# anyboby/Constrained-Model-Based-Policy-Optimization

Hardware: AMD Instinct MI355X
Metric: imagined env-steps/sec (ensemble rollout) + CPO update ms (higher is better)
Workload: dtype f32; 1 GPU; AntSafe-v2 imagined rollout: E=7 x (37->512->512->60) swish ensemble, 5 elites, 3+3 critics 128x128, tanh policy 128x128, B=100000 branches/GPU, maxroll 35 (34 steps), fixed-horizon mode, reset->sample*->finish_all_paths->get(); rollout_mode=schedule, branches_per_gpu=100000, branches_total=100000, horizon=34, task=AntSafe-v2

## Files before the change

constrained-model-based-policy-optimization_amd/csrc/critic_f16.hip:

```cpp
#include "common.h"
#include "ens_mlp_internal.h"
#include "f16_split.h"
#include "policy_f16_tile.h"

namespace {

constexpr int HC = 128;
constexpr int NT = HC / 32;
constexpr int S1 = HC / 16;

struct CfNet {
  const f16x8 *w0, *w1;
  size_t w0_stride, w1_stride;
  const float *b0, *b1, *w2, *b2;
  const float *cst;
  size_t w2_stride;
  const float *stats;
  const float *in_mu, *in_sig, *out_mu, *out_sig;
  float *out;
};

struct CfArgs {
  CfNet net[2];
  const float *obs;
// ... 218 lines not shown
    const int n2 = tid / KP, k = tid - n2 * KP;
    const CfNet &M = a.net[n2];
    const int kc = k < a.obs_dim ? k : 0;
    s_mu[n2 * KP + k] = (M.in_mu && k < a.obs_dim) ? M.in_mu[kc] : 0.0f;
    s_sig[n2 * KP + k] = (M.in_mu && k < a.obs_dim) ? 1.0f / M.in_sig[kc] : 1.0f;
  }
  __syncthreads();
  for (int base = 0; base < tiles * 32 * KP; base += 512 * 4) {
    float xv[4];
    bool ok[4];
#pragma unroll
    for (int u = 0; u < 4; ++u) {
      const int i = base + 512 * u + tid, b = i / KP, k = i - b * KP;
      const int rr = i < tiles * 32 * KP ? rows[b] : -1;
      xv[u] = a.obs[(size_t)(rr >= 0 ? rr : 0) * a.obs_dim + (k < a.obs_dim ? k : 0)];
      ok[u] = rr >= 0 && k < a.obs_dim;
    }
#pragma unroll
    for (int u = 0; u < 4; ++u) {
      const int i = base + 512 * u + tid, b = i / KP, k = i - b * KP;
      if (i < tiles * 32 * KP) xraw[b * XS + k] = ok[u] ? xv[u] : 0.0f;
    }
  }
  for (int net = 0; net < 2 * E; ++net) {
    const int ni = net / E, e = net - ni * E;
    const CfNet &N = a.net[ni];
    __syncthreads();
    {
      const f16x8 *g0 = N.w0 + (size_t)e * N.w0_stride, *g1 = N.w1 + (size_t)e * N.w1_stride;
      constexpr int TOT = G::W0Q + G::W1Q;
      for (int base = 0; base < TOT; base += 512 * 5) {
        f16x8 q[5];
#pragma unroll
        for (int u = 0; u < 5; ++u) {
          const int i = base + 512 * u + tid;
          const int ic = i < TOT ? i : 0;
          q[u] = ic < G::W0Q ? g0[ic] : g1[ic - G::W0Q];
        }
#pragma unroll
        for (int u = 0; u < 5; ++u) {
          const int i = base + 512 * u + tid;
          if (i < TOT) w0s[i] = q[u];
        }
      }
    }
    __syncthreads();
    const float *st = N.stats + (size_t)e * NSTAT;
    const f16x8 *w0 = w0s + lane, *w1 = w1s + lane;
    for (int t = wave; t < tiles; t += 8) {
      const float *xt = xraw + (size_t)t * 32 * XS;
      float xs[S0][8];
      float m0 = 0.0f;
#pragma unroll
      for (int s = 0; s < S0; ++s)
#pragma unroll
        for (int j = 0; j < 8; ++j) {
          const int k = 16 * s + 8 * hh + j;
          float x = (xt[r * XS + k] - s_mu[ni * KP + k]) * s_sig[ni * KP + k];
          if (k >= a.obs_dim) x = 0.0f;
          xs[s][j] = x;
          m0 = fmaxf(m0, fabsf(x));
        }
      m0 = fmaxf(m0, __shfl_xor(m0, 32, 64));
      const float t0 = pow2_lift(m0);
      const float bound1 = (st[1] * m0 + st[2]) * 1.001f, t1 = pow2_lift(bound1);
      const float inv0 = pow2_rcp(st[0] * t0), inv1 = pow2_rcp(st[4] * t1);
      f32x16 acc[NT];
#pragma unroll
      for (int tt = 0; tt < NT; ++tt)
// ... 173 lines not shown
    n.out = outs[i];
  }
  a.obs = d_obs; a.obs_dim = obs_dim; a.ensemble = v->ensemble;
  a.row_idx = d_row_idx; a.n_rows_dev = d_n_rows; a.n_rows = n_rows;
  const int S0 = ms[0]->h3_s0;
  a.has_pol = 0;
  if (policy != nullptr) {
    CMBPO_REQUIRE(cmbpo_internal_critic_pair_can_ride(v, vc, policy) && d_eps && d_pi && d_logp && d_mu && d_ls,
                  "critic pair: the actor cannot ride along (shape / path) or a NULL buffer");
    int ps0 = 0;
    if (int rc = cmbpo_internal_policy_f16_args(policy, &a.pol, &ps0, s)) return rc;
    CMBPO_REQUIRE(ps0 == S0, "critic pair: actor and critics disagree on the input slabs (%d, %d)", ps0, S0);
    a.pol.obs = d_obs; a.pol.eps = d_eps; a.pol.row_idx = d_row_idx; a.pol.n_rows_dev = d_n_rows; a.pol.n_rows = n_rows;
    a.pol.pi = d_pi; a.pol.logp = d_logp; a.pol.mu = d_mu; a.pol.ls = d_ls;
    a.has_pol = 1;
  }
  a.has_store = 0;
  if (store_vec != nullptr) {
    CMBPO_REQUIRE(d_row_idx != nullptr && n_rows < kCriticBigMin && store_vec->fin_code,
                  "critic pair: the store rides with the one-wave-per-member kernel on a row list only");
    a.sv = *store_vec;
    a.has_store = 1;
  }
  if (!a.has_pol && n_rows >= kCriticBigMin) {
    const int n_cu = cmbpo_cu_count();
    auto launch_big = [&](auto geo, auto kern) -> int {
      using G = decltype(geo);
      if (int rc = cmbpo_grant_lds(kern, G::LDS)) return rc;
      int ch = (cmbpo_ceil_div(n_rows, n_cu) + 31) / 32 * 32;
      if (ch > G::CH) ch = G::CH;
      hipLaunchKernelGGL(kern, dim3(cmbpo_ceil_div(n_rows, ch)), dim3(512), G::LDS, s, a, ch);
      CMBPO_HIP_CHECK(hipGetLastError());
      return CMBPO_OK;
    };
    if (S0 == 2) return launch_big(BigGeo<2>{}, critic_big_kernel<2>);
    if (S0 == 3) return launch_big(BigGeo<3>{}, critic_big_kernel<3>);
    return launch_big(BigGeo<4>{}, critic_big_kernel<4>);
  }
  const int threads = 64 * (2 * v->ensemble + a.has_pol);
  const size_t lds = ((size_t)32 * (16 * S0 + 1) + (size_t)2 * v->ensemble * 32) * sizeof(float);
  const int grid = cmbpo_ceil_div(n_rows, 32);
  if (S0 == 2) hipLaunchKernelGGL(critic_pair_kernel<2>, dim3(grid), dim3(threads), lds, s, a);
  else if (S0 == 3) hipLaunchKernelGGL(critic_pair_kernel<3>, dim3(grid), dim3(threads), lds, s, a);
  else hipLaunchKernelGGL(critic_pair_kernel<4>, dim3(grid), dim3(threads), lds, s, a);
  CMBPO_HIP_CHECK(hipGetLastError());
  return CMBPO_OK;
}
// ... 1 lines not shown
```

constrained-model-based-policy-optimization_amd/csrc/policy_f16_tile.h:

```cpp
#pragma once
#include "common.h"
#include "f16_split.h"

namespace {


constexpr int HP = 128;
constexpr int NTP = HP / 32;
constexpr int SP1 = HP / 16;
constexpr float T_H = 16384.0f;

struct PfArgs {
  const f16x8 *w0, *w1, *w2;
  const float *b0, *b1, *b2, *log_std, *stats;
  const float *obs, *eps;
  int obs_dim, act_dim;
  const int32_t *row_idx, *n_rows_dev;
  int n_rows;
  float *pi, *logp, *mu, *ls;
};

__device__ __forceinline__ void tanh_split4(const f32x16 &d, int q, float inv, const f32x4 &bv, unsigned (&q1)[2], unsigned (&q2)[2]) {
  float h[4];
#pragma unroll
  for (int i = 0; i < 4; ++i) h[i] = cmbpo_fast_tanh(__builtin_fmaf(d[4 * q + i], inv, bv[i]));
  split2<true>(h[0], h[1], T_H, q1[0], q2[0]);
  split2<true>(h[2], h[3], T_H, q1[1], q2[1]);
}

struct NoStage { __device__ void operator()() const {} };
template <int S0, bool STAGED, class STAGE = NoStage>
__device__ __forceinline__ void policy_tile(const PfArgs &a, int row0, int n_rows, float *xraw, int *rows, int lane,
                                            STAGE &&stage = STAGE()) {
  constexpr int KP = 16 * S0;
  const int r = lane & 31, hh = lane >> 5;
  const f16x8 *w0 = a.w0 + lane, *w1 = a.w1 + lane, *w2 = a.w2 + lane;
  constexpr int RW = S0 <= 2 ? 3 : 2;
  f16x8 A0[S0][NTP][2], R[3][NTP][2];
  auto load_w = [&](f16x8 (&x)[NTP][2], const f16x8 *w, int slabs, int s) {
#pragma unroll
    for (int t = 0; t < NTP; ++t) {
      const f16x8 *q = w + IMAGE_INDEX(t, slabs, s, 2, 0);
      x[t][0] = q[0]; x[t][1] = q[kImageLanes];
    }
  };
#pragma unroll
  for (int s = 0; s < S0; ++s) load_w(A0[s], w0, S0, s);
#pragma unroll
  for (int s = 0; s < RW; ++s) load_w(R[s], w1, SP1, s);
  if constexpr (!STAGED) {
    if (lane < 32) {
      const int rr = row0 + lane;
      int v = rr < n_rows ? rr : 0;
      if (a.row_idx) v = a.row_idx[v];
      rows[lane] = rr < n_rows ? v : -1;
    }
    __builtin_amdgcn_wave_barrier();
    for (int base = 0; base < 32 * KP; base += 64 * 8) {
      float xv[8];
      bool ok[8];
#pragma unroll
      for (int u = 0; u < 8; ++u) {
        const int i = base + 64 * u + lane, b = i / KP, k = i - b * KP;
        const int rr = rows[b];
        xv[u] = a.obs[(size_t)(rr >= 0 ? rr : 0) * a.obs_dim + (k < a.obs_dim ? k : 0)];
        ok[u] = rr >= 0 && k < a.obs_dim;
      }
#pragma unroll
      for (int u = 0; u < 8; ++u) {
        const int i = base + 64 * u + lane, b = i / KP, k = i - b * KP;
        xraw[b * (KP + 1) + k] = ok[u] ? xv[u] : 0.0f;
      }
// ... 14 lines not shown
      xs[s][j] = x;
      m0 = fmaxf(m0, fabsf(x));
    }
  m0 = fmaxf(m0, __shfl_xor(m0, 32, 64));
  const float t0 = pow2_lift(m0);
  const float inv0 = pow2_rcp(st[0] * t0), inv1 = pow2_rcp(st[4] * T_H), inv2 = pow2_rcp(st[8] * T_H);

  f32x16 acc[NTP];
  auto zero_acc = [&]() {
#pragma unroll
    for (int t = 0; t < NTP; ++t)
#pragma unroll
      for (int i = 0; i < 16; ++i) acc[t][i] = 0.0f;
  };
  zero_acc();
#pragma unroll
  for (int s = 0; s < S0; ++s) {
    unsigned c1[4], c2[4];
#pragma unroll
    for (int j = 0; j < 4; ++j) split2<true>(xs[s][2 * j], xs[s][2 * j + 1], t0, c1[j], c2[j]);
    const u32x4 u1 = {c1[0], c1[1], c1[2], c1[3]}, u2 = {c2[0], c2[1], c2[2], c2[3]};
    const f16x8 b1 = __builtin_bit_cast(f16x8, u1), b2 = __builtin_bit_cast(f16x8, u2);
#pragma unroll
    for (int t = 0; t < NTP; ++t) mm3(acc[t], A0[s][t][0], A0[s][t][1], b1, b2);
  }
  f16x8 bf[SP1][2];
  auto to_frags = [&](const float *bias, float inv) {
    u32x4 bu[SP1][2];
#pragma unroll
    for (int t = 0; t < NTP; ++t)
#pragma unroll
      for (int q = 0; q < 4; ++q) {
        const f32x4 bv = *reinterpret_cast<const f32x4 *>(bias + 32 * t + 8 * q + 4 * hh);
        unsigned q1[2], q2[2];
        tanh_split4(acc[t], q, inv, bv, q1, q2);
        const int S = 2 * t + (q >> 1), o = 2 * (q & 1);
        bu[S][0][o] = q1[0]; bu[S][0][o + 1] = q1[1];
        bu[S][1][o] = q2[0]; bu[S][1][o + 1] = q2[1];
      }
#pragma unroll
    for (int S = 0; S < SP1; ++S) { bf[S][0] = __builtin_bit_cast(f16x8, bu[S][0]); bf[S][1] = __builtin_bit_cast(f16x8, bu[S][1]); }
  };
  to_frags(a.b0, inv0);
  zero_acc();
  if constexpr (RW < 3) load_w(R[2], w1, SP1, 2);
#pragma unroll
  for (int s = 0; s < SP1; ++s) {
#pragma unroll
    for (int t = 0; t < NTP; ++t) mm3(acc[t], R[s % 3][t][0], R[s % 3][t][1], bf[s][0], bf[s][1]);
    if (s + 3 < SP1) load_w(R[s % 3], w1, SP1, s + 3);
  }
  f16x8 W2[SP1][2];
#pragma unroll
  for (int s = 0; s < SP1; ++s) { W2[s][0] = w2[IMAGE_INDEX(0, SP1, s, 2, 0)]; W2[s][1] = w2[IMAGE_INDEX(0, SP1, s, 2, 1)]; }
  to_frags(a.b1, inv1);
  f32x16 o;
#pragma unroll
  for (int i = 0; i < 16; ++i) o[i] = 0.0f;
#pragma unroll
  for (int s = 0; s < SP1; ++s) mm3(o, W2[s][0], W2[s][1], bf[s][0], bf[s][1]);
  const int rr = rows[r];
  const int A = a.act_dim;
  const int nq = (A + 7) >> 3;
  const size_t rbase = (size_t)(rr >= 0 ? rr : 0) * A;
  float lp = 0.0f;
#pragma unroll
  for (int q = 0; q < 4; ++q) {
    if (q < nq) {
      float ev[4], bv[4], lv[4];
#pragma unroll
      for (int e = 0; e < 4; ++e) {
        const int ac = 8 * q + 4 * hh + e, acc = ac < A ? ac : A - 1;
        ev[e] = a.eps[rbase + acc];
// ... 30 lines not shown
```

constrained-model-based-policy-optimization_amd/csrc/rollout_internal.h:

```cpp
#pragma once
#include "common.h"

int cmbpo_internal_book_post_mirror(const cmbpo_rollout_t *r, int n_alive, uint32_t *d_host_out, uint32_t seq, int spec, int min_alive,
                                    double stop_total, void *stream);
int cmbpo_internal_scalars_mirror(const cmbpo_rollout_t *r, uint32_t *d_host_out, uint32_t seq, void *stream);
int cmbpo_internal_book_pre(const cmbpo_rollout_t *r, int n_alive, int spec, int with_vec, void *stream);
int cmbpo_internal_store_nostats(const cmbpo_rollout_t *r, void *stream);
int cmbpo_internal_finish_post_fold(const cmbpo_rollout_t *r, void *stream);
int cmbpo_internal_spec_words(const cmbpo_rollout_t *r, int begin, void *stream);
```

constrained-model-based-policy-optimization_amd/csrc/rollout_state.hip:

```cpp
#include "common.h"
#include "rollout_internal.h"
#include <type_traits>

#include <math.h>

namespace {

constexpr int kScanThreads = 1024;

__device__ __forceinline__ int wave_incl_scan(int v, int lane) {
#pragma unroll
  for (int o = 1; o < 64; o <<= 1) {
    const int t = __shfl_up(v, o, 64);
    if (lane >= o) v += t;
  }
  return v;
}

__device__ __forceinline__ int block_excl_scan(int v, int *sm, int *total) {
  const int lane = threadIdx.x & 63, w = threadIdx.x >> 6, nw = (blockDim.x + 63) >> 6;
  const int inc = wave_incl_scan(v, lane);
  __syncthreads();
  if (lane == 63) sm[w] = inc;
  __syncthreads();
// ... 179 lines not shown
  for (int t = L - 1; t >= 0; --t) {
    const size_t o = (size_t)t * B + b;
    const float rw = r.rew_buf[o], v = r.val_buf[o], c = r.cost_buf[o], cv = r.cval_buf[o];
    double delta;
    if (zero_boot) {
      delta = __dsub_rn(__dadd_rn((double)rw, __dmul_rn(r.gamma, (double)vnext)), (double)v);
    } else {
      delta = (double)__fsub_rn(__fadd_rn(rw, __fmul_rn(g32, vnext)), v);
    }
    const float cdelta = __fsub_rn(__fadd_rn(c, __fmul_rn(cg32, cvnext)), cv);
    y = __dadd_rn(delta, __dmul_rn(gl, y));
    cy = __dadd_rn((double)cdelta, __dmul_rn(cgl, cy));
    const float adv = (float)y, cadv = (float)cy;
    r.adv_buf[o] = adv;
    r.ret_buf[o] = __fadd_rn(adv, v);
    r.cadv_buf[o] = cadv;
    r.cret_buf[o] = __fadd_rn(cadv, cv);
    vnext = v;
    cvnext = cv;
  }
  r.alive[b] = 0;
}

__device__ __forceinline__ void store_stats_body(const cmbpo_rollout_t &r);
__global__ __launch_bounds__(256) void finish_kernel(const cmbpo_rollout_t r, int mode, int fold_stats) {
  if (fold_stats && blockIdx.x == 0) store_stats_body(r);
  const int i = blockIdx.x * blockDim.x + threadIdx.x;
  const int n = r.iscal[CMBPO_I_N_ALIVE];
  if (i >= n) return;
  const int b = r.alive_idx[i];
  float lv, lcv;
  bool zero_boot = false;
  if (mode == 0) {
    const uint8_t code = r.fin_code[b];
    if (!code) return;
    lv = r.v_t[b];
    lcv = r.vc_t[b];
    if (code == 2) {
      lv = 0.0f;
      zero_boot = true;
    }
  } else if (mode == 1) {
    if (r.fin_code[b]) return;
    const bool horizon = (r.ptr + 1 >= r.max_path_length - 1);
    if (horizon) {
      lv = r.v_n[b];
    } else if (r.term_t[b]) {
      lv = 0.0f;
      zero_boot = true;
    } else {
      return;
    }
    lcv = r.vc_n[b];
    atomicAdd(&r.iscal[CMBPO_I_N_FIN_POST], 1);
  } else {
    if (!r.alive[b]) return;
    lv = r.v_t[b];
    lcv = r.vc_t[b];
  }
  gae_finish_path(r, b, lv, lcv, zero_boot);
}

constexpr int kStoreRows = 64;

__global__ __launch_bounds__(256) void store_kernel(const cmbpo_rollout_t r) {
  __shared__ int s_slot[kStoreRows];
  const int n = r.iscal[CMBPO_I_N_ALIVE];
  const int tid = threadIdx.x;
  const int row0 = blockIdx.x * kStoreRows;
  if (row0 >= n) return;
  const size_t B = (size_t)r.B;
  const int D = r.obs_dim, A = r.act_dim;
  if (tid < kStoreRows) {
    double a_cnt = 0, a_cost = 0, a_rew = 0, a_v = 0, a_vc = 0, a_epv = 0, a_maxdkl = 0, a_maxret = 0;
    const int i = row0 + tid;
    int b = -1;
    if (i < n) {
      b = r.alive_idx[i];
      if (r.fin_code[b]) b = -1;
    }
    s_slot[tid] = b;
    if (b >= 0) {
      const size_t col = (size_t)r.ptr * B + b;
      const float rw = r.rew_t[b], c = r.cost_t[b], v = r.v_t[b], vc = r.vc_t[b];
      const float epv = r.epv_t[b], dk = r.dkl_t[b];
      r.rew_buf[col] = rw;
      r.val_buf[col] = v;
      r.cost_buf[col] = c;
      r.cval_buf[col] = vc;
      r.logp_buf[col] = r.logp_t[b];
      r.len[b] = r.ptr + 1;
      const double pr = r.path_ret[b] + (double)rw;
      r.path_ret[b] = pr;
      r.path_cost[b] += (double)c;
      r.path_dyn_var[b] += (double)epv;
      r.dkl_acc[b] += (double)dk;
      a_cnt = 1.0; a_cost = c; a_rew = rw; a_v = v; a_vc = vc;
      a_epv = (double)epv * D;
      a_maxdkl = (double)dk;
      a_maxret = pr;
    }
    const double v0 = wave_sum(a_cnt), v1 = wave_sum(a_cost), v2 = wave_sum(a_rew), v3 = wave_sum(a_v);
    const double v4 = wave_sum(a_vc), v5 = wave_sum(a_epv), v6 = wave_max(a_maxdkl), v7 = wave_max(a_maxret);
    if (tid == 0) {
      double *dst = r.store_part + (size_t)blockIdx.x * 8;
      dst[0] = v0; dst[1] = v1; dst[2] = v2; dst[3] = v3; dst[4] = v4; dst[5] = v5; dst[6] = v6; dst[7] = v7;
    }
  }
  __syncthreads();
  const int rows_here = min(kStoreRows, n - row0);
  const float *vsrc[4] = {r.cur_obs, r.act_t, r.mu_t, r.ls_t};
  float *vdst[4] = {r.obs_buf, r.act_buf, r.mu_buf, r.ls_buf};
  const int vdim[4] = {D, A, A, A};
#pragma unroll
  for (int f = 0; f < 4; ++f) {
    const int dim = vdim[f];
    const float inv = 1.0f / (float)dim;
    for (int e = tid; e < rows_here * dim; e += 256) {
      const int k = (int)(((float)e + 0.5f) * inv);
      const int d = e - k * dim;
      const int b = s_slot[k];
      if (b >= 0) vdst[f][((size_t)r.ptr * B + b) * dim + d] = vsrc[f][(size_t)b * dim + d];
    }
  }
}

__device__ __forceinline__ void store_stats_body(const cmbpo_rollout_t &r) {
  __shared__ double sm_d[16];
  const int n = r.iscal[CMBPO_I_N_ALIVE];
// ... 11 lines not shown
  for (int k = 0; k < 6; ++k) s[k] = block_sum(t[k], sm_d);
  s[6] = block_max(t[6], sm_d);
  s[7] = block_max(t[7], sm_d);
  if (threadIdx.x == 0 && s[0] > 0.0) {
    const double cnt = s[0];
    const double dkl_mean = r.dscal[CMBPO_D_DKL_SUM_T] / (double)n;
    r.iscal[CMBPO_I_N_STORED] += (int)cnt;
    r.iscal[CMBPO_I_SIZE] += (int)cnt;
    r.dscal[CMBPO_D_TOTAL_SAMPLES] += cnt;
    r.dscal[CMBPO_D_TOTAL_COST] += s[1];
    r.dscal[CMBPO_D_TOTAL_REW] += s[2];
    r.dscal[CMBPO_D_SUM_PATH_RET] += s[2];
    r.dscal[CMBPO_D_SUM_PATH_COST] += s[1];
    r.dscal[CMBPO_D_TOTAL_VS] += s[3];
    r.dscal[CMBPO_D_TOTAL_CVS] += s[4];
    r.dscal[CMBPO_D_TOTAL_DYN_EP_VAR] += s[5];
    r.dscal[CMBPO_D_TOTAL_DKL] += dkl_mean * cnt;
    r.dscal[CMBPO_D_MAX_DKL] = fmax(r.dscal[CMBPO_D_MAX_DKL], s[6]);
    r.dscal[CMBPO_D_MAX_PATH_RETURN] = fmax(r.dscal[CMBPO_D_MAX_PATH_RETURN], s[7]);
  }
}

__global__ __launch_bounds__(256) void store_stats_kernel(const cmbpo_rollout_t r) { store_stats_body(r); }

constexpr int kBookMax = 1024;

__global__ __launch_bounds__(kScanThreads) void book_pre_kernel(const cmbpo_rollout_t r, int spec) {
  __shared__ int sm_i[17];
  __shared__ double sm_d[16];
  __shared__ double sm_m[8 * 16];
  __shared__ int s_unc;
  const int tid = threadIdx.x;
  if (spec && r.iscal[CMBPO_I_HALT]) return;
  const int n = r.iscal[CMBPO_I_N_ALIVE];
  {
    double c = 0.0, d = 0.0;
    for (int i = tid; i < n; i += kScanThreads) {
      const int b = r.alive_idx[i];
      const bool u = too_uncertain(r, b);
      r.fin_code[b] = u ? 1 : 0;
      c += u ? 1.0 : 0.0;
      d += (double)r.dkl_t[b];
    }
    double cd[2] = {c, d};
    block_reduce_many<2, 0>(cd, sm_m);
    c = cd[0]; d = cd[1];
// ... 656 lines not shown
extern "C" int cmbpo_rollout_finish(const cmbpo_rollout_t *r, int mode, void *stream) {
  if (int rc = check_rollout(r, "cmbpo_rollout_finish")) return rc;
  CMBPO_REQUIRE(mode >= 0 && mode <= 2, "cmbpo_rollout_finish: bad mode %d", mode);
  CMBPO_REQUIRE(r->rew_buf && r->val_buf && r->cost_buf && r->cval_buf && r->adv_buf && r->ret_buf &&
                    r->cadv_buf && r->cret_buf,
                "cmbpo_rollout_finish: NULL buffer");
  if (mode == 1) CMBPO_REQUIRE(r->v_n && r->vc_n && r->term_t, "cmbpo_rollout_finish: POST needs v_n, vc_n, term_t");
  else CMBPO_REQUIRE(r->v_t && r->vc_t, "cmbpo_rollout_finish: needs v_t, vc_t");
  hipLaunchKernelGGL(finish_kernel, dim3(cmbpo_ceil_div(r->B, 256)), dim3(256), 0, (hipStream_t)stream, *r, mode, 0);
  CMBPO_HIP_CHECK(hipGetLastError());
  return CMBPO_OK;
}

extern "C" int cmbpo_rollout_store(const cmbpo_rollout_t *r, void *stream) {
  if (int rc = check_rollout(r, "cmbpo_rollout_store")) return rc;
  CMBPO_REQUIRE(r->ptr < r->T, "cmbpo_rollout_store: buffer full (ptr %d == T)", r->ptr);
  CMBPO_REQUIRE(r->cur_obs && r->act_t && r->logp_t && r->mu_t && r->ls_t && r->v_t && r->vc_t && r->rew_t &&
                    r->cost_t && r->dkl_t && r->epv_t,
                "cmbpo_rollout_store: NULL step array");
  CMBPO_REQUIRE(r->obs_buf && r->act_buf && r->mu_buf && r->ls_buf && r->rew_buf && r->val_buf && r->cost_buf &&
                    r->cval_buf && r->logp_buf,
                "cmbpo_rollout_store: NULL buffer");
  CMBPO_REQUIRE(r->store_part != nullptr, "cmbpo_rollout_store: NULL store_part scratch");
  hipLaunchKernelGGL(store_kernel, dim3(cmbpo_ceil_div(r->B, kStoreRows)), dim3(256), 0, (hipStream_t)stream, *r);
  hipLaunchKernelGGL(store_stats_kernel, dim3(1), dim3(256), 0, (hipStream_t)stream, *r);
  CMBPO_HIP_CHECK(hipGetLastError());
  return CMBPO_OK;
}

int cmbpo_internal_store_nostats(const cmbpo_rollout_t *r, void *stream) {
  if (int rc = check_rollout(r, "cmbpo_rollout_store")) return rc;
  CMBPO_REQUIRE(r->ptr < r->T, "cmbpo_rollout_store: buffer full (ptr %d == T)", r->ptr);
  CMBPO_REQUIRE(r->cur_obs && r->act_t && r->logp_t && r->mu_t && r->ls_t && r->v_t && r->vc_t && r->rew_t && r->cost_t && r->dkl_t &&
                    r->epv_t && r->obs_buf && r->act_buf && r->mu_buf && r->ls_buf && r->rew_buf && r->val_buf && r->cost_buf &&
                    r->cval_buf && r->logp_buf && r->store_part,
                "cmbpo_rollout_store: NULL array");
  hipLaunchKernelGGL(store_kernel, dim3(cmbpo_ceil_div(r->B, kStoreRows)), dim3(256), 0, (hipStream_t)stream, *r);
  CMBPO_HIP_CHECK(hipGetLastError());
  return CMBPO_OK;
}
int cmbpo_internal_finish_post_fold(const cmbpo_rollout_t *r, void *stream) {
  if (int rc = check_rollout(r, "cmbpo_rollout_finish")) return rc;
  CMBPO_REQUIRE(r->v_n && r->vc_n && r->term_t && r->rew_buf && r->val_buf && r->cost_buf && r->cval_buf && r->adv_buf && r->ret_buf &&
                    r->cadv_buf && r->cret_buf && r->store_part,
                "cmbpo_rollout_finish (POST): NULL array");
  hipLaunchKernelGGL(finish_kernel, dim3(cmbpo_ceil_div(r->B, 256)), dim3(256), 0, (hipStream_t)stream, *r, 1, 1);
  CMBPO_HIP_CHECK(hipGetLastError());
  return CMBPO_OK;
}

extern "C" int cmbpo_rollout_book_pre_max_rows(void) { return kBookMax; }

extern "C" int cmbpo_rollout_book_pre(const cmbpo_rollout_t *r, int n_alive, void *stream) {
  if (int rc = check_rollout(r, "cmbpo_rollout_book_pre")) return rc;
  CMBPO_REQUIRE(n_alive >= 0 && n_alive <= kBookMax, "cmbpo_rollout_book_pre: %d alive rows, at most %d", n_alive, kBookMax);
  CMBPO_REQUIRE(!r->use_host_budget, "cmbpo_rollout_book_pre: the cross-shard budget exchange uses the separate kernels");
  CMBPO_REQUIRE(r->ptr < r->T, "cmbpo_rollout_book_pre: buffer full (ptr %d == T)", r->ptr);
  CMBPO_REQUIRE(r->dkl_t && r->dkl_acc && r->cur_obs && r->act_t && r->logp_t && r->mu_t && r->ls_t && r->v_t && r->vc_t &&
                    r->rew_t && r->cost_t && r->epv_t,
                "cmbpo_rollout_book_pre: NULL step array");
  CMBPO_REQUIRE(r->obs_buf && r->act_buf && r->mu_buf && r->ls_buf && r->rew_buf && r->val_buf && r->cost_buf && r->cval_buf &&
                    r->logp_buf && r->adv_buf && r->ret_buf && r->cadv_buf && r->cret_buf,
                "cmbpo_rollout_book_pre: NULL buffer");
  if (n_alive == 0) return CMBPO_OK;
  hipLaunchKernelGGL(book_pre_kernel, dim3(1), dim3(kScanThreads), 0, (hipStream_t)stream, *r, 0);
  hipLaunchKernelGGL(store_vec_kernel, dim3(cmbpo_ceil_div(n_alive, kStoreRows)), dim3(256), 0, (hipStream_t)stream, *r, 0);
  CMBPO_HIP_CHECK(hipGetLastError());
// ... 12 lines not shown
    hipLaunchKernelGGL(store_vec_kernel, dim3(cmbpo_ceil_div(n_alive, kStoreRows)), dim3(256), 0, (hipStream_t)stream, *r, spec);
  CMBPO_HIP_CHECK(hipGetLastError());
  return CMBPO_OK;
}

__global__ void spec_words_kernel(const cmbpo_rollout_t r, int begin) {
  r.iscal[CMBPO_I_HALT] = 0;
  r.iscal[CMBPO_I_N_EFF] = begin ? r.iscal[CMBPO_I_N_ALIVE] : 0;
}
int cmbpo_internal_spec_words(const cmbpo_rollout_t *r, int begin, void *stream) {
  CMBPO_REQUIRE(r && r->iscal, "look-ahead words: NULL argument");
  hipLaunchKernelGGL(spec_words_kernel, dim3(1), dim3(1), 0, (hipStream_t)stream, *r, begin);
  CMBPO_HIP_CHECK(hipGetLastError());
  return CMBPO_OK;
}

extern "C" int cmbpo_rollout_book_post(const cmbpo_rollout_t *r, int n_alive, void *stream) {
  if (int rc = check_rollout(r, "cmbpo_rollout_book_post")) return rc;
  CMBPO_REQUIRE(n_alive >= 0 && n_alive <= kBookMax, "cmbpo_rollout_book_post: %d alive rows, at most %d", n_alive, kBookMax);
  CMBPO_REQUIRE(r->v_n && r->vc_n && r->term_t && r->rew_buf && r->val_buf && r->cost_buf && r->cval_buf && r->adv_buf &&
                    r->ret_buf && r->cadv_buf && r->cret_buf,
                "cmbpo_rollout_book_post: NULL array");
  hipLaunchKernelGGL(book_post_kernel, dim3(1), dim3(kScanThreads), 0, (hipStream_t)stream, *r, (uint32_t *)nullptr, 0u, 0, 0, 0.0);
  CMBPO_HIP_CHECK(hipGetLastError());
  return CMBPO_OK;
}

__global__ void scalars_mirror_kernel(const cmbpo_rollout_t r, uint32_t *host_out, uint32_t seq) {
  const uint4 *src = reinterpret_cast<const uint4 *>(r.iscal);
  uint4 *dst = reinterpret_cast<uint4 *>(host_out);
  uint4 q[24];
#pragma unroll
  for (int i = 0; i < 24; ++i) q[i] = src[i];
#pragma unroll
  for (int i = 0; i < 24; ++i) dst[i] = q[i];
  __threadfence_system();
  *reinterpret_cast<volatile uint32_t *>(host_out + 96) = seq;
}
int cmbpo_internal_scalars_mirror(const cmbpo_rollout_t *r, uint32_t *d_host_out, uint32_t seq, void *stream) {
  CMBPO_REQUIRE(r && r->iscal && r->dscal && d_host_out, "scalars mirror: NULL argument");
  CMBPO_REQUIRE(reinterpret_cast<const char *>(r->dscal) == reinterpret_cast<const char *>(r->iscal) + 128,
                "scalars mirror: iscal[32] and dscal[32] must be one 384-byte block");
  hipLaunchKernelGGL(scalars_mirror_kernel, dim3(1), dim3(1), 0, (hipStream_t)stream, *r, d_host_out, seq);
  CMBPO_HIP_CHECK(hipGetLastError());
  return CMBPO_OK;
}

int cmbpo_internal_book_post_mirror(const cmbpo_rollout_t *r, int n_alive, uint32_t *d_host_out, uint32_t seq, int spec, int min_alive,
                                    double stop_total, void *stream) {
  if (int rc = check_rollout(r, "cmbpo_rollout_book_post")) return rc;
  CMBPO_REQUIRE(n_alive >= 0 && n_alive <= kBookMax, "cmbpo_rollout_book_post: %d alive rows, at most %d", n_alive, kBookMax);
  CMBPO_REQUIRE(r->v_n && r->vc_n && r->term_t && r->rew_buf && r->val_buf && r->cost_buf && r->cval_buf && r->adv_buf &&
                    r->ret_buf && r->cadv_buf && r->cret_buf,
                "cmbpo_rollout_book_post: NULL array");
  CMBPO_REQUIRE(reinterpret_cast<const char *>(r->dscal) == reinterpret_cast<const char *>(r->iscal) + 128,
                "cmbpo_rollout_book_post: iscal[32] and dscal[32] must be one 384-byte block");
  hipLaunchKernelGGL(book_post_kernel, dim3(1), dim3(kScanThreads), 0, (hipStream_t)stream, *r, d_host_out, seq, spec, min_alive,
                     stop_total);
  CMBPO_HIP_CHECK(hipGetLastError());
  return CMBPO_OK;
}

extern "C" int cmbpo_rollout_read_scalars(const cmbpo_rollout_t *r, void *h_out384, void *stream) {
  CMBPO_REQUIRE(r && r->iscal && r->dscal && h_out384, "cmbpo_rollout_read_scalars: NULL argument");
  CMBPO_REQUIRE(reinterpret_cast<const char *>(r->dscal) == reinterpret_cast<const char *>(r->iscal) + 128,
                "cmbpo_rollout_read_scalars: iscal[32] and dscal[32] must be one 384-byte block");
// ... 115 lines not shown
```

constrained-model-based-policy-optimization_amd/csrc/rollout_step.hip:

```cpp
#include "common.h"
#include "ens_mlp_internal.h"
#include "rollout_internal.h"

#include <string.h>
#include <time.h>

#include <atomic>
#include <mutex>

struct Ahead {
  bool on = false;
  int min_alive = 0;
  double stop_total = 0.0;
};

static int step_impl(const cmbpo_rollout_t *r, int n_alive, cmbpo_mlp_t *policy, cmbpo_mlp_t *model, cmbpo_mlp_t *v,
                     cmbpo_mlp_t *vc, int task, int ensemble, const float *d_eps, const int32_t *d_elite, float *d_mean,
                     float *d_var, bool policy_ready, const float *d_eps_next, bool *next_ready, uint32_t *d_mirror, uint32_t seq,
                     const Ahead &ahead, const float *d_xi, void *stream) {
  CMBPO_REQUIRE(r && policy && model && v && vc && d_eps && d_elite && d_mean && d_var, "cmbpo_rollout_step: NULL argument");
  CMBPO_REQUIRE(n_alive >= 1 && n_alive <= r->B, "cmbpo_rollout_step: n_alive %d not in [1, B=%d]", n_alive, r->B);
  CMBPO_REQUIRE(model->out_dim == r->obs_dim + 1 + ((task & CMBPO_TASK_LEARNED_COST) ? 1 : 0),
                "cmbpo_rollout_step: model out_dim %d does not match obs_dim %d + 1 (+ 1 with CMBPO_TASK_LEARNED_COST), task 0x%x",
                model->out_dim, r->obs_dim, task);
// ... 2 lines not shown
  auto w = [](const float *p) { return const_cast<float *>(p); };
  int rc;
  *next_ready = false;
  const int32_t *d_n = ahead.on ? r->iscal + CMBPO_I_N_EFF : nullptr;
  if (ahead.on)
    CMBPO_REQUIRE(n_alive <= cmbpo_rollout_book_pre_max_rows() && !r->use_host_budget && d_mirror && cmbpo_critic_pair_supported(v, vc),
                  "cmbpo_rollout_run: look-ahead needs the small-batch step");
  if (!policy_ready &&
      (rc = cmbpo_policy_forward(policy, r->cur_obs, r->obs_dim, d_eps, r->alive_idx, d_n, n_alive, w(r->act_t), w(r->logp_t),
                                 w(r->mu_t), w(r->ls_t), stream)))
    return rc;
  if ((rc = cmbpo_ens_forward(model, r->cur_obs, r->obs_dim, r->act_t, r->act_dim, r->alive_idx, d_n, n_alive, r->B,
                              d_mean, d_var, stream)))
    return rc;
  if ((rc = cmbpo_fakeenv_post_noise(task, ensemble, r->obs_dim, r->act_dim, d_mean, d_var, r->B, r->cur_obs, r->act_t, d_elite,
                                     r->alive_idx, d_n, n_alive, w(r->next_obs), w(r->rew_t), const_cast<uint8_t *>(r->term_t),
                                     w(r->cost_t), w(r->dkl_t), w(r->epv_t), nullptr, d_xi, stream)))
    return rc;
  const bool small = ahead.on || (n_alive <= cmbpo_rollout_book_pre_max_rows() && !r->use_host_budget);
  const bool vec_rides = small && cmbpo_critic_pair_supported(v, vc) && n_alive < kCriticBigMin;
  if (small) {
    if ((rc = cmbpo_internal_book_pre(r, n_alive, ahead.on ? 1 : 0, vec_rides ? 0 : 1, stream))) return rc;
  } else {
    const bool fold_late = !r->use_host_budget;
    if ((rc = cmbpo_rollout_decide(r, stream))) return rc;
    if (r->uncertainty_mode || r->max_samples != 0 || r->use_host_budget)
      if ((rc = cmbpo_rollout_finish(r, 0, stream))) return rc;
    if ((rc = fold_late ? cmbpo_internal_store_nostats(r, stream) : cmbpo_rollout_store(r, stream))) return rc;
  }
  if (cmbpo_critic_pair_supported(v, vc)) {
    const bool ride = d_eps_next != nullptr && n_alive < kCriticBigMin &&
                      cmbpo_internal_critic_pair_can_ride(v, vc, policy);
    CmbpoStoreVec sv{};
    if (vec_rides) {
      const float *src[4] = {r->cur_obs, r->act_t, r->mu_t, r->ls_t};
      float *dst[4] = {r->obs_buf, r->act_buf, r->mu_buf, r->ls_buf};
      const int dim[4] = {r->obs_dim, r->act_dim, r->act_dim, r->act_dim};
      for (int f = 0; f < 4; ++f) { sv.src[f] = src[f]; sv.dst[f] = dst[f]; sv.dim[f] = dim[f]; }
      sv.fin_code = r->fin_code;
      sv.col_off = (size_t)r->ptr * (size_t)r->B;
    }
    if ((rc = cmbpo_internal_critic_pair_ride(v, vc, r->next_obs, r->obs_dim, r->alive_idx, d_n, n_alive, w(r->v_n), w(r->vc_n),
                                              ride ? policy : nullptr, d_eps_next, w(r->act_t), w(r->logp_t), w(r->mu_t), w(r->ls_t),
                                              stream, vec_rides ? &sv : nullptr)))
      return rc;
    *next_ready = ride;
  } else {
    if ((rc = cmbpo_ens_predict_mean(v, r->next_obs, r->obs_dim, r->alive_idx, nullptr, n_alive, w(r->v_n), stream))) return rc;
    if ((rc = cmbpo_ens_predict_mean(vc, r->next_obs, r->obs_dim, r->alive_idx, nullptr, n_alive, w(r->vc_n), stream))) return rc;
  }
  if (small) {
    if ((rc = d_mirror ? cmbpo_internal_book_post_mirror(r, n_alive, d_mirror, seq, ahead.on ? 1 : 0, ahead.min_alive, ahead.stop_total,
                                                         stream)
                       : cmbpo_rollout_book_post(r, n_alive, stream)))
      return rc;
    return 1;
  }
  return r->use_host_budget ? cmbpo_rollout_finish(r, 1, stream) : cmbpo_internal_finish_post_fold(r, stream);
}

extern "C" int cmbpo_rollout_step(const cmbpo_rollout_t *r, int n_alive, cmbpo_mlp_t *policy, cmbpo_mlp_t *model,
                                  cmbpo_mlp_t *v, cmbpo_mlp_t *vc, int task, int ensemble, const float *d_eps,
                                  const int32_t *d_elite, float *d_mean, float *d_var, void *stream) {
  bool unused = false;
  return step_impl(r, n_alive, policy, model, v, vc, task, ensemble, d_eps, d_elite, d_mean, d_var, false, nullptr, &unused, nullptr, 0u,
                   Ahead{}, r ? r->xi : nullptr, stream);
}

namespace {
constexpr int kMirrorSlots = 64, kMirrorDwords = 128, kMaxDevices = 64;
struct Mirror {
  uint32_t *h = nullptr, *d = nullptr;
  bool tried = false;
};
Mirror g_mirror[kMaxDevices];
std::mutex g_mirror_mu;
std::atomic<uint32_t> g_seq{0};

uint32_t next_seq() {
  uint32_t s = g_seq.fetch_add(1, std::memory_order_relaxed) + 1;
  return s ? s : g_seq.fetch_add(1, std::memory_order_relaxed) + 1;
// ... 101 lines not shown
        cur = nxt;
      }
      if (halted)
        if (int rc = cmbpo_internal_spec_words(r, 0, stream)) return rc;
      break;
    }
    const float *eps_next = done + 1 < max_steps ? d_eps + (size_t)(done + 1) * eps_stride : nullptr;
    bool next_ready = false;
    const int slot = done % kMirrorSlots;
    const uint32_t seq = next_seq();
    uint32_t *d_slot = mir.d ? mir.d + (size_t)slot * kMirrorDwords : nullptr;
    int rc = step_impl(r, n_alive, policy, model, v, vc, task, ensemble, d_eps + (size_t)done * eps_stride,
                       d_elite + (size_t)done * elite_stride, d_mean, d_var, ready, eps_next, &next_ready, d_slot, seq, Ahead{},
                       xi_at(done), stream);
    ready = next_ready;
    if (rc != 0 && rc != 1) return rc;
    char *h = static_cast<char *>(h_scalars) + (size_t)done * 384;
    if (rc == 1 && d_slot != nullptr) {
      const uint32_t *h_slot = mir.h + (size_t)slot * kMirrorDwords;
      if (int rc2 = wait_mirror(h_slot, seq, (hipStream_t)stream)) return rc2;
      memcpy(h, h_slot, 384);
    } else if (d_slot != nullptr) {
      const uint32_t *h_slot = mir.h + (size_t)slot * kMirrorDwords;
      if (int rc2 = cmbpo_internal_scalars_mirror(r, d_slot, seq, stream)) return rc2;
      if (eps_next != nullptr && !ready && r->ptr + 1 < r->T) {
        auto w = [](const float *q) { return const_cast<float *>(q); };
        if (int rc2 = cmbpo_policy_forward(policy, r->next_obs, r->obs_dim, eps_next, r->alive_idx, nullptr, n_alive, w(r->act_t),
                                           w(r->logp_t), w(r->mu_t), w(r->ls_t), stream))
          return rc2;
        ready = true;
      }
      if (int rc2 = wait_mirror(h_slot, seq, (hipStream_t)stream)) return rc2;
      memcpy(h, h_slot, 384);
    } else if (int rc2 = cmbpo_rollout_read_scalars(r, h, stream)) {
      return rc2;
    }
    const int32_t *isc = reinterpret_cast<const int32_t *>(h);
    const double *dsc = reinterpret_cast<const double *>(h + 128);
    const int fin = isc[CMBPO_I_N_FIN_PRE] + isc[CMBPO_I_N_FIN_POST];
    bool swap_lists = rc == 1;
    if (rc == 0 && fin > 0) {
      if (int rc2 = cmbpo_rollout_compact(r, stream)) return rc2;
      swap_lists = true;
    }
    n_alive -= fin;
    advance(swap_lists);
    ++done;
// ... 9 lines not shown
```

constrained-model-based-policy-optimization_amd/modelbuffer.py:

```python
import ctypes as C

import numpy as np
import torch

from . import _lib
from ._lib import RolloutStruct

EPS = 1e-8


def _np_or_t(x, device, dtype=torch.float32):
    if isinstance(x, torch.Tensor):
        return x.to(device=device, dtype=dtype)
    return torch.as_tensor(np.ascontiguousarray(x), device=device).to(dtype)


class ModelBuffer:
    def __init__(self, batch_size, obs_dim, act_dim, max_path_length, device=None, comm=None,
                 *args, **kwargs):
        self.max_path_length = int(max_path_length)
        self.batch_size = int(batch_size)
        self.capacity = int(batch_size)
        self.obs_shape, self.act_shape = obs_dim, act_dim
        self.obs_dim = int(np.prod(obs_dim))
# ... 5 lines not shown
        self._alloc(self.capacity)
        self.reset()

    def _alloc(self, B):
        T, D, A, dev = self.max_path_length, self.obs_dim, self.act_dim, self.device
        f = dict(dtype=torch.float32, device=dev)
        d = dict(dtype=torch.float64, device=dev)
        t = {}
        for name, dim in (("obs_buf", D), ("act_buf", A), ("mu_buf", A), ("ls_buf", A)):
            t[name] = torch.empty((T, B, dim), **f)
        for name in ("rew_buf", "val_buf", "cost_buf", "cval_buf", "logp_buf",
                     "adv_buf", "ret_buf", "cadv_buf", "cret_buf"):
            t[name] = torch.empty((T, B), **f)
        t["alive_idx"] = torch.empty(B, dtype=torch.int32, device=dev)
        t["alive_idx_out"] = torch.empty(B, dtype=torch.int32, device=dev)
        t["scal_bytes"] = torch.zeros(32 * 4 + 32 * 8, dtype=torch.uint8, device=dev)
        t["iscal"] = t["scal_bytes"][:128].view(torch.int32)
        t["dscal"] = t["scal_bytes"][128:].view(torch.float64)
        t["alive"] = torch.empty(B, dtype=torch.uint8, device=dev)
        t["fin_code"] = torch.empty(B, dtype=torch.uint8, device=dev)
        t["len"] = torch.empty(B, dtype=torch.int32, device=dev)
        for name in ("dkl_acc", "path_ret", "path_cost", "path_dyn_var"):
            t[name] = torch.empty(B, **d)
        t["store_part"] = torch.empty(((B + 63) // 64) * 8, **d)
        for name, dim in (("cur_obs", D), ("next_obs", D), ("act_t", A), ("mu_t", A), ("ls_t", A)):
            t[name] = torch.zeros((B, dim), **f)
        for name in ("logp_t", "v_t", "vc_t", "v_n", "vc_n", "rew_t", "cost_t", "dkl_t", "epv_t"):
            t[name] = torch.zeros(B, **f)
        t["term_t"] = torch.zeros(B, dtype=torch.uint8, device=dev)
        t["offsets"] = torch.empty(B + 1, dtype=torch.int32, device=dev)
        t["stats"] = torch.zeros(16, **d)
        self.t = t
        self.capacity = B
        self.rs = RolloutStruct()
        self.rs.T, self.rs.obs_dim, self.rs.act_dim = T, D, A
        self.rs.rank, self.rs.world = 0, 1
        self.rs.max_samples = 0
        self.rs.dkl_lim = float("inf")
        self.rs.max_path_length = T
        self._bind_all()

    def _bind_all(self):
        for name, _ in RolloutStruct._fields_:
            if name in self.t:
                setattr(self.rs, name, self.t[name].data_ptr())
        self.rs.use_host_budget = 0

# ... 156 lines not shown
```

Measured before the change: 71.57 million imagined env-steps/s.

## Ride policy forward in big critic kernel and fold scalar mirror into store

New measurement: 69.91 million imagined env-steps/s. 0.977x the previous value.

```diff
diff --git a/constrained-model-based-policy-optimization_amd/csrc/critic_f16.hip b/constrained-model-based-policy-optimization_amd/csrc/critic_f16.hip
--- a/constrained-model-based-policy-optimization_amd/csrc/critic_f16.hip
+++ b/constrained-model-based-policy-optimization_amd/csrc/critic_f16.hip
@@ -264,12 +264,13 @@
       if (i < tiles * 32 * KP) xraw[b * XS + k] = ok[u] ? xv[u] : 0.0f;
     }
   }
-  for (int net = 0; net < 2 * E; ++net) {
-    const int ni = net / E, e = net - ni * E;
+  for (int net = 0; net < 2 * E + a.has_pol; ++net) {
+    const bool is_pol = net == 2 * E;
+    const int ni = is_pol ? 0 : net / E, e = is_pol ? 0 : net - ni * E;
     const CfNet &N = a.net[ni];
     __syncthreads();
     {
-      const f16x8 *g0 = N.w0 + (size_t)e * N.w0_stride, *g1 = N.w1 + (size_t)e * N.w1_stride;
+      const f16x8 *g0 = is_pol ? a.pol.w0 : N.w0 + (size_t)e * N.w0_stride, *g1 = is_pol ? a.pol.w1 : N.w1 + (size_t)e * N.w1_stride;
       constexpr int TOT = G::W0Q + G::W1Q;
       for (int base = 0; base < TOT; base += 512 * 5) {
         f16x8 q[5];
@@ -287,6 +288,12 @@
       }
     }
     __syncthreads();
+    if (is_pol) {
+      for (int t = wave; t < tiles; t += 8)
+        policy_tile<S0, true, NoStage, true>(a.pol, row0 + t * 32, n_rows, xraw + (size_t)t * 32 * XS, rows + t * 32, lane, NoStage(),
+                                             w0s, w1s);
+      break;
+    }
     const float *st = N.stats + (size_t)e * NSTAT;
     const f16x8 *w0 = w0s + lane, *w1 = w1s + lane;
     for (int t = wave; t < tiles; t += 8) {
@@ -506,7 +513,7 @@
     a.sv = *store_vec;
     a.has_store = 1;
   }
-  if (!a.has_pol && n_rows >= kCriticBigMin) {
+  if (n_rows >= kCriticBigMin) {
     const int n_cu = cmbpo_cu_count();
     auto launch_big = [&](auto geo, auto kern) -> int {
       using G = decltype(geo);
diff --git a/constrained-model-based-policy-optimization_amd/csrc/policy_f16_tile.h b/constrained-model-based-policy-optimization_amd/csrc/policy_f16_tile.h
--- a/constrained-model-based-policy-optimization_amd/csrc/policy_f16_tile.h
+++ b/constrained-model-based-policy-optimization_amd/csrc/policy_f16_tile.h
@@ -29,12 +29,12 @@
 }
 
 struct NoStage { __device__ void operator()() const {} };
-template <int S0, bool STAGED, class STAGE = NoStage>
+template <int S0, bool STAGED, class STAGE = NoStage, bool WLDS = false>
 __device__ __forceinline__ void policy_tile(const PfArgs &a, int row0, int n_rows, float *xraw, int *rows, int lane,
-                                            STAGE &&stage = STAGE()) {
+                                            STAGE &&stage = STAGE(), const f16x8 *lds_w0 = nullptr, const f16x8 *lds_w1 = nullptr) {
   constexpr int KP = 16 * S0;
   const int r = lane & 31, hh = lane >> 5;
-  const f16x8 *w0 = a.w0 + lane, *w1 = a.w1 + lane, *w2 = a.w2 + lane;
+  const f16x8 *w0 = (WLDS ? lds_w0 : a.w0) + lane, *w1 = (WLDS ? lds_w1 : a.w1) + lane, *w2 = a.w2 + lane;
   constexpr int RW = S0 <= 2 ? 3 : 2;
   f16x8 A0[S0][NTP][2], R[3][NTP][2];
   auto load_w = [&](f16x8 (&x)[NTP][2], const f16x8 *w, int slabs, int s) {
@@ -44,10 +44,12 @@
       x[t][0] = q[0]; x[t][1] = q[kImageLanes];
     }
   };
-#pragma unroll
-  for (int s = 0; s < S0; ++s) load_w(A0[s], w0, S0, s);
-#pragma unroll
-  for (int s = 0; s < RW; ++s) load_w(R[s], w1, SP1, s);
+  if constexpr (!WLDS) {
+#pragma unroll
+    for (int s = 0; s < S0; ++s) load_w(A0[s], w0, S0, s);
+#pragma unroll
+    for (int s = 0; s < RW; ++s) load_w(R[s], w1, SP1, s);
+  }
   if constexpr (!STAGED) {
     if (lane < 32) {
       const int rr = row0 + lane;
@@ -108,7 +110,14 @@
     const u32x4 u1 = {c1[0], c1[1], c1[2], c1[3]}, u2 = {c2[0], c2[1], c2[2], c2[3]};
     const f16x8 b1 = __builtin_bit_cast(f16x8, u1), b2 = __builtin_bit_cast(f16x8, u2);
 #pragma unroll
-    for (int t = 0; t < NTP; ++t) mm3(acc[t], A0[s][t][0], A0[s][t][1], b1, b2);
+    for (int t = 0; t < NTP; ++t) {
+      if constexpr (WLDS) {
+        const f16x8 *q = w0 + IMAGE_INDEX(t, S0, s, 2, 0);
+        mm3(acc[t], q[0], q[kImageLanes], b1, b2);
+      } else {
+        mm3(acc[t], A0[s][t][0], A0[s][t][1], b1, b2);
+      }
+    }
   }
   f16x8 bf[SP1][2];
   auto to_frags = [&](const float *bias, float inv) {
@@ -129,12 +138,22 @@
   };
   to_frags(a.b0, inv0);
   zero_acc();
-  if constexpr (RW < 3) load_w(R[2], w1, SP1, 2);
-#pragma unroll
-  for (int s = 0; s < SP1; ++s) {
-#pragma unroll
-    for (int t = 0; t < NTP; ++t) mm3(acc[t], R[s % 3][t][0], R[s % 3][t][1], bf[s][0], bf[s][1]);
-    if (s + 3 < SP1) load_w(R[s % 3], w1, SP1, s + 3);
+  if constexpr (WLDS) {
+#pragma unroll
+    for (int s = 0; s < SP1; ++s)
+#pragma unroll
+      for (int t = 0; t < NTP; ++t) {
+        const f16x8 *q = w1 + IMAGE_INDEX(t, SP1, s, 2, 0);
+        mm3(acc[t], q[0], q[kImageLanes], bf[s][0], bf[s][1]);
+      }
+  } else {
+    if constexpr (RW < 3) load_w(R[2], w1, SP1, 2);
+#pragma unroll
+    for (int s = 0; s < SP1; ++s) {
+#pragma unroll
+      for (int t = 0; t < NTP; ++t) mm3(acc[t], R[s % 3][t][0], R[s % 3][t][1], bf[s][0], bf[s][1]);
+      if (s + 3 < SP1) load_w(R[s % 3], w1, SP1, s + 3);
+    }
   }
   f16x8 W2[SP1][2];
 #pragma unroll
diff --git a/constrained-model-based-policy-optimization_amd/csrc/rollout_internal.h b/constrained-model-based-policy-optimization_amd/csrc/rollout_internal.h
--- a/constrained-model-based-policy-optimization_amd/csrc/rollout_internal.h
+++ b/constrained-model-based-policy-optimization_amd/csrc/rollout_internal.h
@@ -3,8 +3,7 @@
 
 int cmbpo_internal_book_post_mirror(const cmbpo_rollout_t *r, int n_alive, uint32_t *d_host_out, uint32_t seq, int spec, int min_alive,
                                     double stop_total, void *stream);
-int cmbpo_internal_scalars_mirror(const cmbpo_rollout_t *r, uint32_t *d_host_out, uint32_t seq, void *stream);
 int cmbpo_internal_book_pre(const cmbpo_rollout_t *r, int n_alive, int spec, int with_vec, void *stream);
-int cmbpo_internal_store_nostats(const cmbpo_rollout_t *r, void *stream);
-int cmbpo_internal_finish_post_fold(const cmbpo_rollout_t *r, void *stream);
+int cmbpo_internal_store_fold(const cmbpo_rollout_t *r, uint32_t *d_host_out, uint32_t seq, void *stream);
+int cmbpo_internal_finish_post_counted(const cmbpo_rollout_t *r, void *stream);
 int cmbpo_internal_spec_words(const cmbpo_rollout_t *r, int begin, void *stream);
diff --git a/constrained-model-based-policy-optimization_amd/csrc/rollout_state.hip b/constrained-model-based-policy-optimization_amd/csrc/rollout_state.hip
--- a/constrained-model-based-policy-optimization_amd/csrc/rollout_state.hip
+++ b/constrained-model-based-policy-optimization_amd/csrc/rollout_state.hip
@@ -225,9 +225,7 @@
   r.alive[b] = 0;
 }
 
-__device__ __forceinline__ void store_stats_body(const cmbpo_rollout_t &r);
-__global__ __launch_bounds__(256) void finish_kernel(const cmbpo_rollout_t r, int mode, int fold_stats) {
-  if (fold_stats && blockIdx.x == 0) store_stats_body(r);
+__global__ __launch_bounds__(256) void finish_kernel(const cmbpo_rollout_t r, int mode, int counted) {
   const int i = blockIdx.x * blockDim.x + threadIdx.x;
   const int n = r.iscal[CMBPO_I_N_ALIVE];
   if (i >= n) return;
@@ -255,7 +253,7 @@
       return;
     }
     lcv = r.vc_n[b];
-    atomicAdd(&r.iscal[CMBPO_I_N_FIN_POST], 1);
+    if (!counted) atomicAdd(&r.iscal[CMBPO_I_N_FIN_POST], 1);
   } else {
     if (!r.alive[b]) return;
     lv = r.v_t[b];
@@ -266,7 +264,7 @@
 
 constexpr int kStoreRows = 64;
 
-__global__ __launch_bounds__(256) void store_kernel(const cmbpo_rollout_t r) {
+__global__ __launch_bounds__(256) void store_kernel(const cmbpo_rollout_t r, int fin_part) {
   __shared__ int s_slot[kStoreRows];
   const int n = r.iscal[CMBPO_I_N_ALIVE];
   const int tid = threadIdx.x;
@@ -275,7 +273,7 @@
   const size_t B = (size_t)r.B;
   const int D = r.obs_dim, A = r.act_dim;
   if (tid < kStoreRows) {
-    double a_cnt = 0, a_cost = 0, a_rew = 0, a_v = 0, a_vc = 0, a_epv = 0, a_maxdkl = 0, a_maxret = 0;
+    double a_cnt = 0, a_cost = 0, a_rew = 0, a_v = 0, a_vc = 0, a_epv = 0, a_maxdkl = 0, a_maxret = 0, a_fin = 0;
     const int i = row0 + tid;
     int b = -1;
     if (i < n) {
@@ -284,6 +282,7 @@
     }
     s_slot[tid] = b;
     if (b >= 0) {
+      if (fin_part) a_fin = (r.ptr + 1 >= r.max_path_length - 1 || r.term_t[b]) ? 1.0 : 0.0;
       const size_t col = (size_t)r.ptr * B + b;
       const float rw = r.rew_t[b], c = r.cost_t[b], v = r.v_t[b], vc = r.vc_t[b];
       const float epv = r.epv_t[b], dk = r.dkl_t[b];
@@ -308,6 +307,10 @@
     if (tid == 0) {
       double *dst = r.store_part + (size_t)blockIdx.x * 8;
       dst[0] = v0; dst[1] = v1; dst[2] = v2; dst[3] = v3; dst[4] = v4; dst[5] = v5; dst[6] = v6; dst[7] = v7;
+    }
+    if (fin_part) {
+      const double v8 = wave_sum(a_fin);
+      if (tid == 0) r.store_part[(size_t)gridDim.x * 8 + blockIdx.x] = v8;
     }
   }
   __syncthreads();
@@ -365,6 +368,30 @@
 }
 
 __global__ __launch_bounds__(256) void store_stats_kernel(const cmbpo_rollout_t r) { store_stats_body(r); }
+
+__global__ __launch_bounds__(256) void store_fold_kernel(const cmbpo_rollout_t r, int n_tiles_max, uint32_t *host_out, uint32_t seq) {
+  __shared__ double sm_f[16];
+  store_stats_body(r);
+  const int n = r.iscal[CMBPO_I_N_ALIVE];
+  const int n_wg = (n + kStoreRows - 1) / kStoreRows;
+  double f = 0.0;
+  for (int w = threadIdx.x; w < n_wg; w += 256) f += r.store_part[(size_t)n_tiles_max * 8 + w];
+  f = block_sum(f, sm_f);
+  if (threadIdx.x == 0) {
+    r.iscal[CMBPO_I_N_FIN_POST] = (int)f;
+    if (host_out != nullptr) {
+      const uint4 *src = reinterpret_cast<const uint4 *>(r.iscal);
+      uint4 *dst = reinterpret_cast<uint4 *>(host_out);
+      uint4 q[24];
+#pragma unroll
+      for (int i = 0; i < 24; ++i) q[i] = src[i];
+#pragma unroll
+      for (int i = 0; i < 24; ++i) dst[i] = q[i];
+      __threadfence_system();
+      *reinterpret_cast<volatile uint32_t *>(host_out + 96) = seq;
+    }
+  }
+}
 
 constexpr int kBookMax = 1024;
 
@@ -1067,27 +1094,31 @@
                     r->cval_buf && r->logp_buf,
                 "cmbpo_rollout_store: NULL buffer");
   CMBPO_REQUIRE(r->store_part != nullptr, "cmbpo_rollout_store: NULL store_part scratch");
-  hipLaunchKernelGGL(store_kernel, dim3(cmbpo_ceil_div(r->B, kStoreRows)), dim3(256), 0, (hipStream_t)stream, *r);
+  hipLaunchKernelGGL(store_kernel, dim3(cmbpo_ceil_div(r->B, kStoreRows)), dim3(256), 0, (hipStream_t)stream, *r, 0);
   hipLaunchKernelGGL(store_stats_kernel, dim3(1), dim3(256), 0, (hipStream_t)stream, *r);
   CMBPO_HIP_CHECK(hipGetLastError());
   return CMBPO_OK;
 }
 
-int cmbpo_internal_store_nostats(const cmbpo_rollout_t *r, void *stream) {
+int cmbpo_internal_store_fold(const cmbpo_rollout_t *r, uint32_t *d_host_out, uint32_t seq, void *stream) {
   if (int rc = check_rollout(r, "cmbpo_rollout_store")) return rc;
   CMBPO_REQUIRE(r->ptr < r->T, "cmbpo_rollout_store: buffer full (ptr %d == T)", r->ptr);
   CMBPO_REQUIRE(r->cur_obs && r->act_t && r->logp_t && r->mu_t && r->ls_t && r->v_t && r->vc_t && r->rew_t && r->cost_t && r->dkl_t &&
-                    r->epv_t && r->obs_buf && r->act_buf && r->mu_buf && r->ls_buf && r->rew_buf && r->val_buf && r->cost_buf &&
-                    r->cval_buf && r->logp_buf && r->store_part,
+                    r->epv_t && r->term_t && r->obs_buf && r->act_buf && r->mu_buf && r->ls_buf && r->rew_buf && r->val_buf &&
+                    r->cost_buf && r->cval_buf && r->logp_buf && r->store_part,
                 "cmbpo_rollout_store: NULL array");
-  hipLaunchKernelGGL(store_kernel, dim3(cmbpo_ceil_div(r->B, kStoreRows)), dim3(256), 0, (hipStream_t)stream, *r);
-  CMBPO_HIP_CHECK(hipGetLastError());
-  return CMBPO_OK;
-}
-int cmbpo_internal_finish_post_fold(const cmbpo_rollout_t *r, void *stream) {
+  CMBPO_REQUIRE(reinterpret_cast<const char *>(r->dscal) == reinterpret_cast<const char *>(r->iscal) + 128,
+                "cmbpo_rollout_store: iscal[32] and dscal[32] must be one 384-byte block");
+  const int tiles = cmbpo_ceil_div(r->B, kStoreRows);
+  hipLaunchKernelGGL(store_kernel, dim3(tiles), dim3(256), 0, (hipStream_t)stream, *r, 1);
+  hipLaunchKernelGGL(store_fold_kernel, dim3(1), dim3(256), 0, (hipStream_t)stream, *r, tiles, d_host_out, seq);
+  CMBPO_HIP_CHECK(hipGetLastError());
+  return CMBPO_OK;
+}
+int cmbpo_internal_finish_post_counted(const cmbpo_rollout_t *r, void *stream) {
   if (int rc = check_rollout(r, "cmbpo_rollout_finish")) return rc;
   CMBPO_REQUIRE(r->v_n && r->vc_n && r->term_t && r->rew_buf && r->val_buf && r->cost_buf && r->cval_buf && r->adv_buf && r->ret_buf &&
-                    r->cadv_buf && r->cret_buf && r->store_part,
+                    r->cadv_buf && r->cret_buf,
                 "cmbpo_rollout_finish (POST): NULL array");
   hipLaunchKernelGGL(finish_kernel, dim3(cmbpo_ceil_div(r->B, 256)), dim3(256), 0, (hipStream_t)stream, *r, 1, 1);
   CMBPO_HIP_CHECK(hipGetLastError());
@@ -1146,26 +1177,6 @@
                     r->ret_buf && r->cadv_buf && r->cret_buf,
                 "cmbpo_rollout_book_post: NULL array");
   hipLaunchKernelGGL(book_post_kernel, dim3(1), dim3(kScanThreads), 0, (hipStream_t)stream, *r, (uint32_t *)nullptr, 0u, 0, 0, 0.0);
-  CMBPO_HIP_CHECK(hipGetLastError());
-  return CMBPO_OK;
-}
-
-__global__ void scalars_mirror_kernel(const cmbpo_rollout_t r, uint32_t *host_out, uint32_t seq) {
-  const uint4 *src = reinterpret_cast<const uint4 *>(r.iscal);
-  uint4 *dst = reinterpret_cast<uint4 *>(host_out);
-  uint4 q[24];
-#pragma unroll
-  for (int i = 0; i < 24; ++i) q[i] = src[i];
-#pragma unroll
-  for (int i = 0; i < 24; ++i) dst[i] = q[i];
-  __threadfence_system();
-  *reinterpret_cast<volatile uint32_t *>(host_out + 96) = seq;
-}
-int cmbpo_internal_scalars_mirror(const cmbpo_rollout_t *r, uint32_t *d_host_out, uint32_t seq, void *stream) {
-  CMBPO_REQUIRE(r && r->iscal && r->dscal && d_host_out, "scalars mirror: NULL argument");
-  CMBPO_REQUIRE(reinterpret_cast<const char *>(r->dscal) == reinterpret_cast<const char *>(r->iscal) + 128,
-                "scalars mirror: iscal[32] and dscal[32] must be one 384-byte block");
-  hipLaunchKernelGGL(scalars_mirror_kernel, dim3(1), dim3(1), 0, (hipStream_t)stream, *r, d_host_out, seq);
   CMBPO_HIP_CHECK(hipGetLastError());
   return CMBPO_OK;
 }
diff --git a/constrained-model-based-policy-optimization_amd/csrc/rollout_step.hip b/constrained-model-based-policy-optimization_amd/csrc/rollout_step.hip
--- a/constrained-model-based-policy-optimization_amd/csrc/rollout_step.hip
+++ b/constrained-model-based-policy-optimization_amd/csrc/rollout_step.hip
@@ -48,15 +48,13 @@
   if (small) {
     if ((rc = cmbpo_internal_book_pre(r, n_alive, ahead.on ? 1 : 0, vec_rides ? 0 : 1, stream))) return rc;
   } else {
-    const bool fold_late = !r->use_host_budget;
     if ((rc = cmbpo_rollout_decide(r, stream))) return rc;
     if (r->uncertainty_mode || r->max_samples != 0 || r->use_host_budget)
       if ((rc = cmbpo_rollout_finish(r, 0, stream))) return rc;
-    if ((rc = fold_late ? cmbpo_internal_store_nostats(r, stream) : cmbpo_rollout_store(r, stream))) return rc;
+    if ((rc = r->use_host_budget ? cmbpo_rollout_store(r, stream) : cmbpo_internal_store_fold(r, d_mirror, seq, stream))) return rc;
   }
   if (cmbpo_critic_pair_supported(v, vc)) {
-    const bool ride = d_eps_next != nullptr && n_alive < kCriticBigMin &&
-                      cmbpo_internal_critic_pair_can_ride(v, vc, policy);
+    const bool ride = d_eps_next != nullptr && cmbpo_internal_critic_pair_can_ride(v, vc, policy);
     CmbpoStoreVec sv{};
     if (vec_rides) {
       const float *src[4] = {r->cur_obs, r->act_t, r->mu_t, r->ls_t};
@@ -82,7 +80,7 @@
       return rc;
     return 1;
   }
-  return r->use_host_budget ? cmbpo_rollout_finish(r, 1, stream) : cmbpo_internal_finish_post_fold(r, stream);
+  return r->use_host_budget ? cmbpo_rollout_finish(r, 1, stream) : cmbpo_internal_finish_post_counted(r, stream);
 }
 
 extern "C" int cmbpo_rollout_step(const cmbpo_rollout_t *r, int n_alive, cmbpo_mlp_t *policy, cmbpo_mlp_t *model,
@@ -230,7 +228,6 @@
       memcpy(h, h_slot, 384);
     } else if (d_slot != nullptr) {
       const uint32_t *h_slot = mir.h + (size_t)slot * kMirrorDwords;
-      if (int rc2 = cmbpo_internal_scalars_mirror(r, d_slot, seq, stream)) return rc2;
       if (eps_next != nullptr && !ready && r->ptr + 1 < r->T) {
         auto w = [](const float *q) { return const_cast<float *>(q); };
         if (int rc2 = cmbpo_policy_forward(policy, r->next_obs, r->obs_dim, eps_next, r->alive_idx, nullptr, n_alive, w(r->act_t),
diff --git a/constrained-model-based-policy-optimization_amd/modelbuffer.py b/constrained-model-based-policy-optimization_amd/modelbuffer.py
--- a/constrained-model-based-policy-optimization_amd/modelbuffer.py
+++ b/constrained-model-based-policy-optimization_amd/modelbuffer.py
@@ -51,7 +51,7 @@
         t["len"] = torch.empty(B, dtype=torch.int32, device=dev)
         for name in ("dkl_acc", "path_ret", "path_cost", "path_dyn_var"):
             t[name] = torch.empty(B, **d)
-        t["store_part"] = torch.empty(((B + 63) // 64) * 8, **d)
+        t["store_part"] = torch.empty(((B + 63) // 64) * 9, **d)
         for name, dim in (("cur_obs", D), ("next_obs", D), ("act_t", A), ("mu_t", A), ("ls_t", A)):
             t[name] = torch.zeros((B, dim), **f)
         for name in ("logp_t", "v_t", "vc_t", "v_n", "vc_n", "rew_t", "cost_t", "dkl_t", "epv_t"):
```
